# Ascend-Research/HeadPoseEstimation-WHENet

Measured on AMD Instinct MI355X. Metric: head crops/sec (224x224), higher is better.
Workload: dtype f16

## Files before the change

__graft_entry__.py:

```python
from __future__ import annotations

import os
import subprocess
import sys
from concurrent.futures import ThreadPoolExecutor

ROOT = os.path.dirname(os.path.abspath(__file__))
PKG = os.path.join(ROOT, "headposeestimation-whenet_amd")
CSRC = os.path.join(PKG, "csrc")
LIBDIR = os.path.join(PKG, "lib")
OBJDIR = os.path.join(PKG, "build")
LIB = os.path.join(LIBDIR, "libwhenet_hip.so")

SOURCES = ["stem.hip", "stemdw.hip", "dw.hip", "se.hip", "pw.hip", "head.hip", "head7.hip", "front.hip", "front2.hip", "front2s.hip", "front7.hip", "mb7.hip", "frame.hip", "yolo.hip", "convert.hip",
           "snapshot.cpp", "engine.cpp", "engine_post.cpp", "engine_ops.cpp", "capi.cpp"]
HEADERS = ["common.h", "spec.h", "snapshot.h", "kernels.h", "device_math.h", "engine.h", "engine_internal.h", "stamps.h", "se_device.h", "front_tuned_f16.inc", "front_tuned_f32.inc", "front2_tuned.inc", "front2s_tuned.inc",
           os.path.join("..", "..", "include", "whenet_hip.h")]
EXTRA_FLAGS = {"front2.hip": ["-mllvm", "-amdgpu-mfma-vgpr-form"], "front2s.hip": ["-mllvm", "-amdgpu-mfma-vgpr-form"], "front7.hip": ["-mllvm", "-amdgpu-mfma-vgpr-form"],
               "mb7.hip": ["-mllvm", "-amdgpu-mfma-vgpr-form"]}
CXXFLAGS = ["--offload-arch=gfx950", "-mcode-object-version=5", "-O3", "-std=c++17", "-fPIC", "-Wall",
            "-Wno-unused-function", "-fvisibility=hidden"]


def _hipcc() -> str:
    for cand in (os.environ.get("HIPCC"), "/opt/rocm/bin/hipcc", "hipcc"):
        if cand and (os.path.isabs(cand) and os.path.exists(cand) or not os.path.isabs(cand)):
            return cand
    raise RuntimeError("hipcc not found")


def _stale(target: str, deps) -> bool:
    if not os.path.exists(target):
        return True
    t = os.path.getmtime(target)
    return any(os.path.getmtime(d) > t for d in deps if os.path.exists(d))


def build(force: bool = False, verbose: bool = False) -> None:
    os.makedirs(LIBDIR, exist_ok=True)
    os.makedirs(OBJDIR, exist_ok=True)
    hipcc = _hipcc()
    hdrs = [os.path.join(CSRC, h) for h in HEADERS]

    def compile_one(src: str) -> str:
        s = os.path.join(CSRC, src)
        o = os.path.join(OBJDIR, src.replace(".", "_") + ".o")
        if force or _stale(o, [s] + hdrs):
            cmd = [hipcc] + CXXFLAGS + EXTRA_FLAGS.get(src, []) + ["-c", s, "-o", o]
            if verbose:
                print(" ".join(cmd), flush=True)
            r = subprocess.run(cmd, capture_output=True, text=True)
            if r.returncode != 0:
                raise RuntimeError(f"hipcc failed on {src}:\n{r.stdout}\n{r.stderr}")
        return o

    with ThreadPoolExecutor(max_workers=min(8, len(SOURCES))) as ex:
        objs = list(ex.map(compile_one, SOURCES))
    if force or _stale(LIB, objs):
        cmd = [hipcc, "--offload-arch=gfx950", "-shared", "-fPIC", "-o", LIB] + objs + \
              ["-Wl,-rpath,/opt/rocm/lib", "-Wl,--no-undefined"]
        if verbose:
            print(" ".join(cmd), flush=True)
        r = subprocess.run(cmd, capture_output=True, text=True)
        if r.returncode != 0:
            raise RuntimeError(f"link failed:\n{r.stdout}\n{r.stderr}")
    if PKG not in sys.path:
        sys.path.insert(0, PKG)
    import whenet
    from whenet_hip import _lib
    _lib.load()

# ... 55 lines not shown
```

headposeestimation-whenet_amd/csrc/engine.cpp:

```cpp
#include "engine_internal.h"

#include <mutex>

#include <algorithm>
#include <cstdlib>
#include <cmath>
#include <cstring>

namespace whenet {

using namespace detail;

void* Engine::upload_bytes(const void* p, size_t nbytes) {
    void* d = nullptr;
    WHENET_HIP_CHECK(hipMalloc(&d, nbytes ? nbytes : 16));
    weight_allocs_.push_back(d);
    if (nbytes) WHENET_HIP_CHECK(hipMemcpy(d, p, nbytes, hipMemcpyHostToDevice));
    return d;
}

template <typename T> T* Engine::upload(const std::vector<T>& v) {
    return static_cast<T*>(upload_bytes(v.data(), v.size() * sizeof(T)));
}

// ... 36 lines not shown
    for (const HostBlock& hb : m.blocks) {
        DevBlock b;
        b.spec = hb.spec;
        if (hb.spec.has_expand()) b.expand = upload_pw(hb.expand);
        b.dw.k = hb.dw.k;
        b.dw.C = hb.dw.C;
        b.dw.w = upload(hb.dw.w);
        b.dw.bias = upload(hb.dw.bias);
        b.dw.plan = plan_dw(dtype_, hb.spec.k, hb.spec.s, hb.spec.h_in, hb.spec.h_out, hb.dw.C);
        b.se.C = hb.se.C;
        b.se.R = hb.se.R;
        b.se.w1t = upload(hb.se.w1t);
        b.se.b1 = upload(hb.se.b1);
        b.se.w2 = upload(hb.se.w2);
        b.se.w2c = upload(hb.se.w2c);
        b.se.b2 = upload(hb.se.b2);
        if (split_ && !hb.se.excite.packed_split.empty()) {
            b.se.w2p = upload_bytes(hb.se.excite.packed_split.data(), hb.se.excite.packed_split.size());
            b.se.KSr = hb.se.excite.KS_split;
            b.se.w2_wsi = hb.se.excite.wsi;
        } else if (dtype_ == WHENET_F16 && !hb.se.excite.packed.empty()) {
            b.se.w2p = upload_bytes(hb.se.excite.packed.data(), hb.se.excite.packed.size());
            b.se.KSr = hb.se.excite.KS;
        }
        b.project = upload_pw(hb.project);
        partial_per_crop_ = std::max(partial_per_crop_, size_t(b.dw.plan.ntiles()) * b.dw.C);
        if (hb.spec.has_expand()) {
            b.fplan = plan_front(dtype_, hb.spec.k, hb.spec.s, hb.spec.h_in, hb.spec.h_out, hb.dw.C);
            partial_per_crop_ = std::max(partial_per_crop_, size_t(b.fplan.ntiles()) * b.dw.C);
            partial_per_crop_ = std::max(partial_per_crop_, size_t(b.fplan.ntiles()) * size_t(b.fplan.chunks) *
                                                                size_t(se_padded_r(b.se.R)));
            if (dtype_ == WHENET_F16) {
                b.f2plan = plan_front2(hb.spec.k, hb.spec.s, hb.spec.h_in, hb.spec.h_out, hb.dw.C);
                b.f2_preferred = front2_preferred(hb.spec.k, hb.spec.s, hb.spec.h_in, hb.dw.C);
                b.dw.wt = upload(pack_dw_toeplitz(hb.dw.w, hb.spec.k, hb.spec.s, hb.dw.C, b.f2plan.xs));
                partial_per_crop_ = std::max(partial_per_crop_, size_t(b.f2plan.ntiles()) * b.dw.C);
                partial_per_crop_ = std::max(partial_per_crop_, size_t(b.f2plan.ntiles()) * size_t(b.f2plan.chunks) *
                                                                    size_t(se_padded_r(b.se.R)));
            }
            if (split_ && front2s_supported(hb.spec.k, hb.spec.s, hb.spec.h_in, hb.spec.cin)) {
                b.f2s_supported = true;
                b.f2splan = plan_front2s(hb.spec.k, hb.spec.s, hb.spec.h_in, hb.spec.h_out, hb.dw.C, &b.f2s_tm);
                b.f2s_preferred = front2s_preferred(hb.spec.k, hb.spec.s, hb.spec.h_in, hb.dw.C);
                b.dw.wts = upload(pack_dw_toeplitz_s(hb.dw.w, hb.spec.k, hb.spec.s, hb.dw.C, b.f2s_tm, &b.dw.wts_wsi));
                partial_per_crop_ = std::max(partial_per_crop_, size_t(b.f2splan.ntiles()) * size_t(b.f2splan.chunks) *
                                                                    size_t(se_padded_r(b.se.R)));
            }
            b.f7_supported = front7_supported(hb.spec.k, hb.spec.s, hb.spec.h_in, hb.spec.cin);
            if (b.f7_supported) {
                if (dtype_ == WHENET_F16) b.dw.wt7 = upload(pack_dw_toeplitz(hb.dw.w, hb.spec.k, 1, hb.dw.C, 4 - hb.spec.k / 2));
                b.f7_chunks = front7_plan_for(dtype_, hb.spec.cin, hb.dw.C, 64).chunks;
                partial_per_crop_ = std::max(partial_per_crop_, size_t(b.f7_chunks) * size_t(se_padded_r(b.se.R)));
            }
        }
        if (mb7_supported(dtype_, hb.spec.k, hb.spec.s, hb.spec.h_in, hb.spec.cin, hb.dw.C, hb.se.R, hb.spec.cout, hb.spec.has_skip())) {
            std::vector<half_t> w1p, w2p;
            pack_mb7_se(hb.se.w1t, hb.se.w2, hb.se.C, hb.se.R, &w1p, &w2p);
            b.mb7.wds = upload(pack_mb7_taps(hb.dw.w, hb.spec.k, hb.dw.C));
            b.mb7.w1p = upload(w1p);
            b.mb7.w2p = upload(w2p);
            b.mb7.ok = true;
        }
        blocks_.push_back(b);
    }
    head_ = upload_pw(m.head);
    fold12_pw_ = upload_pw(m.fold12);
    d_fold12_w32_ = upload(m.fold12_w32);
    d_dense_w_ = upload(m.dense_w);
    d_dense_b_ = upload(m.dense_b);
    WHENET_HIP_CHECK(hipDeviceSynchronize());
}

void Engine::open_device(int device_id) {
    int count = 0;
    hipError_t e = hipGetDeviceCount(&count);
    if (e != hipSuccess || count <= 0)
        throw Error(WHENET_ENODEV, std::string("no HIP device visible (") + hipGetErrorString(e) +
                                       "); libwhenet_hip has no CPU fallback");
    WHENET_REQUIRE(device_id >= 0 && device_id < count, WHENET_ENODEV,
                   "device_id " + std::to_string(device_id) + " out of range (" + std::to_string(count) + " devices)");
    DeviceGuard guard(device_id);
    WHENET_HIP_CHECK(hipGetDeviceProperties(&prop_, device_id));
    WHENET_REQUIRE(std::strstr(prop_.gcnArchName, "gfx950") != nullptr, WHENET_ENODEV,
                   std::string("device is ") + prop_.gcnArchName + "; this library carries gfx950 code only");
    num_cus_ = prop_.multiProcessorCount;

    WHENET_HIP_CHECK(hipStreamCreateWithFlags(&stream_, hipStreamNonBlocking));
    WHENET_HIP_CHECK(hipEventCreateWithFlags(&fork_ev_, hipEventDisableTiming));
    for (int i = 0; i < MAX_LANES - 1; ++i) {
        hipEvent_t ev = nullptr;
        WHENET_HIP_CHECK(hipEventCreateWithFlags(&ev, hipEventDisableTiming));
        join_ev_.push_back(ev);
    }
}

Engine::Engine(int device_id) : device_(device_id), dtype_(WHENET_F32) { open_device(device_id); }

void Engine::require_model() const {
    WHENET_REQUIRE(has_model_, WHENET_EINVAL, "this handle was created without a network (whenet_create_postproc)");
}

Engine::~Engine() {
    (void)hipSetDevice(device_);
    if (stream_) (void)hipStreamSynchronize(stream_);
    if (copy_stream_) (void)hipStreamSynchronize(copy_stream_);
    for (auto& kv : graphs_) (void)hipGraphExecDestroy(kv.second);
// ... 19 lines not shown
    if (hout_ypr_) (void)hipHostFree(hout_ypr_);
    if (hout_amax_) (void)hipHostFree(hout_amax_);
    if (hout_logits_) (void)hipHostFree(hout_logits_);
    void* arena[] = {x0_, x1_, e_, d_, hc_, partial_, gate_, hcount_, in_u8_, o_ypr_, o_amax_, o_logits_, in_f32_, yolo_scratch_};
    for (void* p : arena)
        if (p) (void)hipFree(p);
    for (void* p : weight_allocs_) (void)hipFree(p);
    for (hipStream_t st : lane_streams_) { (void)hipStreamSynchronize(st); (void)hipStreamDestroy(st); }
    for (hipEvent_t ev : join_ev_) (void)hipEventDestroy(ev);
    if (fork_ev_) (void)hipEventDestroy(fork_ev_);
    if (stream_) (void)hipStreamDestroy(stream_);
    if (copy_stream_) (void)hipStreamDestroy(copy_stream_);
}

void Engine::set_option(const std::string& key, long value) {
    DeviceGuard guard(device_);
    if (key == "graph") {
        use_graph_ = value != 0;
    } else if (key == "pw_impl") {
        WHENET_REQUIRE(value == 0 || value == 1, WHENET_EINVAL, "pw_impl must be 0 (MFMA) or 1 (check kernel)");
        pw_impl_ = int(value);
        sync();
        drop_graphs();
    } else if (key == "fuse_front") {
        fuse_front_ = value != 0;
        sync();
        drop_graphs();
    } else if (key == "se_fuse") {
        WHENET_REQUIRE(value >= 0 && value <= 3, WHENET_EINVAL,
                       "se_fuse must be 0 (never), 1 (where the prologue form pays), 2 (prologue form on every block) or 3 (1 + the matrix-core form on blocks 7-16, default)");
        se_fuse_ = int(value);
        sync();
        drop_graphs();
    } else if (key == "front_impl") {
        WHENET_REQUIRE(value >= 0 && value <= 2, WHENET_EINVAL,
                       "front_impl must be 0 (front.hip everywhere), 1 (per layer, default) or 2 (front2.hip / front2s.hip wherever they exist)");
        front_impl_ = int(value);
        sync();
        drop_graphs();
    } else if (key == "f2s_mask") {
        WHENET_REQUIRE(value >= -1 && value < (1 << 17), WHENET_EINVAL, "f2s_mask must be -1 or a bit mask of blocks 2..12");
        f2s_mask_ = int(value);
        sync();
        drop_graphs();
    } else if (key == "head_fuse") {
        head_fuse_ = value != 0;
        sync();
        drop_graphs();
    } else if (key == "concurrent") {
        xcd_always_ = value != 0;
        sync();
        drop_graphs();
    } else if (key == "xcd_map") {
        WHENET_REQUIRE(value >= 0 && value <= 7, WHENET_EINVAL, "xcd_map must be a bit mask 0..7 (1 = front / front2, 2 = front7, 4 = head7)");
        xcd_map_ = int(value);
        sync();
        drop_graphs();
    } else if (key == "mb7") {
        mb7_ = value != 0;
        sync();
        drop_graphs();
    } else if (key == "front7") {
        front7_ = value != 0;
        sync();
        drop_graphs();
    } else if (key == "fold12") {
        fold12_ = value != 0;
        sync();
        drop_graphs();
    } else if (key == "stem_fuse") {
        stem_fuse_ = value != 0;
        sync();
        drop_graphs();
    } else if (key == "poison") {
        poison_ = value != 0;
    } else if (key == "lanes" || key == "device_lanes") {
        WHENET_REQUIRE(value >= 1 && value <= MAX_LANES, WHENET_EINVAL, "lanes must be 1..8");
        lanes_ = int(value);
        if (key == "lanes") host_lanes_ = int(value);
        sync();
        drop_graphs();
    } else if (key == "split_heads") {
        split_heads_ = value != 0;
        sync();
        drop_graphs();
    } else if (key == "lane_graphs") {
        lane_graphs_ = value != 0;
        sync();
        drop_graphs();
    } else if (key == "pw_staged") {
        pw_staged_ = value != 0;
        sync();
        drop_graphs();
    } else if (key == "split_pw") {
        WHENET_REQUIRE(split_ || value == 0, WHENET_EINVAL, "split_pw: the handle was not created as WHENET_F32S");
        split_pw_ = value != 0;
        sync();
        drop_graphs();
    } else if (key == "host_pinned_max") {
        WHENET_REQUIRE(value >= 0 && value <= 4096, WHENET_EINVAL, "host_pinned_max must be 0..4096");
        sync();
        host_pinned_max_ = int(value);
    } else if (key == "se_fuse_tiny") {
        WHENET_REQUIRE(value >= 0 && value <= 64, WHENET_EINVAL, "se_fuse_tiny must be 0..64");
        se_fuse_tiny_ = int(value);
        sync();
        drop_graphs();
    } else if (key == "host_lanes") {
        WHENET_REQUIRE(value >= 1 && value <= MAX_LANES, WHENET_EINVAL, "host_lanes must be 1..8");
        host_lanes_ = int(value);
    } else if (key == "min_lane_crops") {
        WHENET_REQUIRE(value >= 1, WHENET_EINVAL, "min_lane_crops must be >= 1");
        min_lane_crops_ = int(value);
        sync();
        drop_graphs();
    } else if (key == "repeat") {
// ... 74 lines not shown
    x1_ = alloc(N * X_ELEMS * es);
    e_ = alloc(N * E_ELEMS * es);
    d_ = alloc(N * D_ELEMS * es);
    hc_ = alloc(N * HC_ELEMS * es);
    partial_ = static_cast<float*>(alloc(N * partial_per_crop_ * sizeof(float)));
    gate_ = static_cast<float*>(alloc(N * 1152 * sizeof(float)));
    hcount_ = static_cast<unsigned*>(alloc(N * sizeof(unsigned)));
    WHENET_HIP_CHECK(hipMemsetAsync(hcount_, 0, N * sizeof(unsigned), stream_));
    WHENET_HIP_CHECK(hipStreamSynchronize(stream_));
    in_u8_ = static_cast<uint8_t*>(alloc(N * IN_BYTES));
    o_ypr_ = static_cast<float*>(alloc(N * 3 * sizeof(float)));
    o_amax_ = static_cast<int32_t*>(alloc(N * 3 * sizeof(int32_t)));
    o_logits_ = static_cast<float*>(alloc(N * N_LOGITS * sizeof(float)));
    cap_ = n;
    arena_bytes_ = total;
}

namespace {

struct Rec {
    LaunchRecorder* rec;
    hipStream_t s;
    int repeat = 1;
    template <typename F>
    void operator()(const std::string& layer, const char* kind, const std::string& kernel, double bytes, double flops,
                    F&& fn) {
        if (!rec) {
            for (int i = 0; i < repeat; ++i) fn();
            return;
        }
        if (rec->first_pass) {
            LaunchRecorder::Entry e;
            e.layer = layer;
            e.kind = kind;
            e.kernel = kernel;
            e.bytes = bytes;
            e.flops = flops;
            WHENET_HIP_CHECK(hipEventCreate(&e.stop));
            rec->entries.push_back(e);
        }
        LaunchRecorder::Entry& e = rec->entries.at(rec->cursor++);
        fn();
        WHENET_HIP_CHECK(hipEventRecord(e.stop, s));
    }
};

}

Engine::BlockSchedule Engine::block_schedule(const DevBlock& b, int n) const {
    BlockSchedule r;
    r.fused = fuse_front_ && b.spec.has_expand() && pw_impl_ == 0;
    r.use_f7 = r.fused && front_impl_ == 1 && front7_ && b.f7_supported;
    r.use_mb7 = r.use_f7 && mb7_ && dtype_ == WHENET_F16 && b.mb7.ok;
    r.use_f2 = r.fused && !r.use_f7 && dtype_ == WHENET_F16 && (front_impl_ == 2 || (front_impl_ == 1 && b.f2_preferred));
    const bool f2s_pick = f2s_mask_ >= 0 ? ((f2s_mask_ >> b.spec.index) & 1) != 0 : b.f2s_preferred;
    r.use_f2s = r.fused && !r.use_f7 && split_ && split_pw_ && b.f2s_supported && b.expand.wps != nullptr &&
                (front_impl_ == 2 || (front_impl_ == 1 && f2s_pick));
    r.se_in_front = r.fused;
    r.se_ntiles = r.use_f7 ? 1 : (r.use_f2 ? b.f2plan.ntiles() : (r.use_f2s ? b.f2splan.ntiles() : (r.fused ? b.fplan.ntiles() : b.dw.plan.ntiles())));
    r.se_chunks = r.use_f7 ? b.f7_chunks : (r.use_f2 ? b.f2plan.chunks : (r.use_f2s ? b.f2splan.chunks : b.fplan.chunks));
    const bool se_pays = b.project.K < 320 && r.se_ntiles * r.se_chunks <= 24;
    const bool tiny = !single_stage_call_ && n > 0 && n <= se_fuse_tiny_ && b.project.K < 1152;
    r.se_mfma = r.se_in_front && pw_impl_ == 0 && se_fuse_ == 3 && pw_staged_ && b.project.K >= 320 && b.se.w2p != nullptr &&
                (dtype_ == WHENET_F16 || (split_ && split_pw_));
    r.se_fused = r.se_in_front && pw_impl_ == 0 && (se_fuse_ == 2 || r.se_mfma || ((se_fuse_ == 1 || se_fuse_ == 3) && (se_pays || tiny)));
    return r;
}

bool Engine::fold12_active() const {
    if (!(fold12_ && fuse_front_ && pw_impl_ == 0 && blocks_.size() >= 2)) return false;
    if (dtype_ == WHENET_F16) return front_impl_ == 2 || (front_impl_ == 1 && blocks_[1].f2_preferred);
    const BlockSchedule b2 = block_schedule(blocks_[1]);
    return split_ && split_pw_ && fold12_pw_.wps != nullptr && b2.fused && !b2.use_f2s && !b2.use_f7;
}

bool Engine::stem_fuse_active() const {
    if (!(stem_fuse_ && !blocks_.empty())) return false;
    const DevBlock& b = blocks_[0];
    return !b.spec.has_expand() && !b.spec.has_skip() &&
           stemdw_supported(dtype_, b.dw.plan, b.spec.k, b.spec.s, b.spec.h_in, b.spec.cexp());
}

void* Engine::enqueue_blocks(int first, int last, const View& v, void* cur, int n, hipStream_t s, LaunchRecorder* rec,
                             bool b1_dw_done) {
    const bool fold = fold12_active() && first <= 1 && last >= 2;
    for (int i = first; i <= last; ++i) {
        void* nxt = (cur == v.x0) ? v.x1 : v.x0;
        enqueue_block(blocks_[size_t(i - 1)], v, cur, nxt, n, s, rec, fold && i <= 2 ? i : 0, b1_dw_done && i == 1);
        cur = nxt;
    }
    return cur;
}

void Engine::enqueue_block(const DevBlock& b, const View& v, const void* in, void* out, int n, hipStream_t s,
                           LaunchRecorder* rec, int fold, bool dw_done) {
    Rec R{rec, s, repeat_};
    const BlockSpec& sp = b.spec;
    const std::string p = "b" + std::to_string(sp.index);
    const double es = double(esz());
    const int hw_in = sp.h_in * sp.h_in, hw_out = sp.h_out * sp.h_out;
    const int cexp = sp.cexp();
    const void* dw_in = in;
    const BlockSchedule bs = block_schedule(b, n);
    const bool fused = bs.fused, use_f2 = bs.use_f2, se_in_front = bs.se_in_front, se_fused = bs.se_fused;
    const int se_ntiles = bs.se_ntiles, se_chunks = bs.se_chunks;
    WHENET_REQUIRE(fold == 0 || (fold == 1 && !fused && sp.index == 1) ||
                       (fold == 2 && sp.index == 2 && (use_f2 || (split_ && fused && !bs.use_f2s && !bs.use_f7))), WHENET_EINVAL,
                   "fold12: block outside the folded pair");
    if (bs.use_mb7) {
        WHENET_REQUIRE(fold == 0, WHENET_EINVAL, "mb7: block outside the 7 x 7 stage");
        Mb7Args a{};
        a.x = in;
        a.wep = b.expand.wp;
        a.be = b.expand.bias;
        a.wds = b.mb7.wds;
        a.bd = b.dw.bias;
        a.w1p = b.mb7.w1p;
        a.b1 = b.se.b1;
        a.w2p = b.mb7.w2p;
        a.b2 = b.se.b2;
        a.wpp = b.project.wp;
        a.bp = b.project.bias;
        a.out = out;
        if (single_stage_call_) {
            a.dbg_dw = v.d;
            a.dbg_gate = v.gate;
        }
        a.k = sp.k;
        a.Cout = sp.cout;
        a.skip = sp.has_skip();
        a.n = n;
        R(p + "/mbconv", "mbconv", kernel_name_mb7(sp.k, sp.cout, a.skip).c_str(),
          double(n) * (hw_in * sp.cin * (a.skip ? 2 : 1) + hw_out * sp.cout) * es,
          2.0 * n * (double(hw_in) * sp.cin * cexp + double(hw_out) * sp.k * sp.k * cexp + double(hw_out) * cexp * sp.cout),
          [&] { launch_mb7(a, s); });
        return;
    }
    if (bs.use_f7) {
        Front7Args a{};
        a.dtype = dtype_;
        a.x = in;
        a.wep = b.expand.wp;
        a.be = b.expand.bias;
        a.wdt = dtype_ == WHENET_F16 ? static_cast<const void*>(b.dw.wt7) : static_cast<const void*>(b.dw.w);
        a.bd = b.dw.bias;
        a.out = v.d;
        a.rpart = v.partial;
        a.w1t = b.se.w1t;
        a.R = b.se.R;
        a.k = sp.k;
        a.Cin = sp.cin;
        a.Cexp = cexp;
        a.NTe = b.expand.NTILES;
        a.split = split_ && split_pw_ && b.expand.wps != nullptr;
        a.weps = b.expand.wps;
        a.wsi = b.expand.wsi;
        a.n = n;
        a.xcd_grouped = xcd_grouped(2, n);
        a.plan = front7_plan_for(dtype_, sp.cin, cexp, n);
        R(p + "/front", "front", kernel_name_front7(dtype_, sp.k, a.plan, a.split).c_str(), double(n) * (hw_in * sp.cin + hw_out * cexp) * es,
          2.0 * n * (double(hw_in) * sp.cin * cexp + double(hw_out) * sp.k * sp.k * cexp), [&] { launch_front7(a, s); });
    } else if (use_f2) {
        Front2Args a{};
        a.x = in;
        a.wep = b.expand.wp;
        a.be = b.expand.bias;
        a.wdt = b.dw.wt;
        a.bd = b.dw.bias;
        a.out = v.d;
        a.rpart = v.partial;
        a.w1t = b.se.w1t;
        a.R = b.se.R;
        a.k = sp.k;
        a.s = sp.s;
        a.H = sp.h_in;
        a.Ho = sp.h_out;
        a.Cin = sp.cin;
        a.Cexp = cexp;
        a.pad = sp.pad_before();
        a.KSe = b.expand.KS;
        a.NTe = b.expand.NTILES;
        if (fold == 2) {
            a.wep = d_fold12_w32_;
            a.be = fold12_pw_.bias;
            a.Cin = fold12_pw_.K;
            a.KSe = fold12_pw_.KS;
            a.NTe = fold12_pw_.NTILES;
            a.in_gate = static_cast<const float*>(v.gate);
        }
        a.n = n;
        a.xcd_grouped = xcd_grouped(1, n);
        a.plan = b.f2plan;
        a.plan.threads = front2_threads(b.f2plan, n);
        R(p + "/front", "front", kernel_name_front2(sp.k, sp.s, a.KSe, a.plan.threads, a.plan.xs, a.in_gate != nullptr).c_str(),
          double(n) * (hw_in * a.Cin + hw_out * cexp) * es,
          2.0 * n * (double(hw_in) * a.Cin * cexp + double(hw_out) * sp.k * sp.k * cexp), [&] { launch_front2(a, s); });
    } else if (bs.use_f2s) {
        Front2sArgs a{};
        a.x = in;
        a.weps = b.expand.wps;
        a.be = b.expand.bias;
        a.wdt = b.dw.wts;
        a.bd = b.dw.bias;
        a.out = v.d;
        a.rpart = v.partial;
        a.w1t = b.se.w1t;
        a.R = b.se.R;
        a.k = sp.k;
        a.s = sp.s;
        a.H = sp.h_in;
        a.Ho = sp.h_out;
        a.Cin = sp.cin;
        a.Cexp = cexp;
        a.pad = sp.pad_before();
// ... 668 lines not shown
```

headposeestimation-whenet_amd/csrc/engine.h:

```cpp
#pragma once

#include <map>
#include <memory>
#include <string>
#include <tuple>
#include <vector>

#include "common.h"
#include "kernels.h"
#include "snapshot.h"

namespace whenet {

struct DevPw {
    int K = 0, N = 0, KS = 0, NTILES = 0;
    void* wp = nullptr;
    void* wps = nullptr;
    int KSs = 0;
    float wsi = 1.0f;
    float* wdense = nullptr;
    float* bias = nullptr;
};
struct DevDw {
    int k = 0, C = 0;
    float* w = nullptr;
    float* bias = nullptr;
    half_t* wt = nullptr;
    half_t* wt7 = nullptr;
    float* wts = nullptr;
    float wts_wsi = 1.0f;
    DwPlan plan;
};
struct DevSe {
    int C = 0, R = 0;
    float *w1t = nullptr, *b1 = nullptr, *w2 = nullptr, *b2 = nullptr;
    float* w2c = nullptr;
    void* w2p = nullptr;
    int KSr = 0;
    float w2_wsi = 1.0f;
};
struct DevMb7 {
    bool ok = false;
    half_t *wds = nullptr, *w1p = nullptr, *w2p = nullptr;
};
struct DevBlock {
    BlockSpec spec;
    DevPw expand;
    DevDw dw;
    FrontPlan fplan;
    Front2Plan f2plan;
    bool f2_preferred = false;
    Front2Plan f2splan;
    int f2s_tm = 2;
    bool f2s_supported = false, f2s_preferred = false;
    bool f7_supported = false;
    int f7_chunks = 1;
    DevSe se;
    DevPw project;
    DevMb7 mb7;
};

struct LaunchRecorder {
    struct Entry {
        std::string layer, kind, kernel;
        double bytes = 0, flops = 0;
        hipEvent_t stop = nullptr;
        double total_ms = 0;
    };
    std::vector<Entry> entries;
    hipEvent_t start = nullptr;
    size_t cursor = 0;
    bool first_pass = true;
};

constexpr int MAX_LANES = 8;

class Engine {
  public:
    Engine(const void* snapshot, size_t nbytes, int device_id, int dtype);
    explicit Engine(int device_id);
    ~Engine();
    Engine(const Engine&) = delete;
    Engine& operator=(const Engine&) = delete;

    void set_option(const std::string& key, long value);
    void get_info(whenet_info_t* out) const;

    void forward_host(const uint8_t* crops, int n, float* ypr, int32_t* argmax, float* logits);
    void forward_host_f32(const float* x, int n, float* ypr, int32_t* argmax, float* logits);
    void forward_device(const uint8_t* d_crops, int n, float* d_ypr, int32_t* d_argmax, float* d_logits,
                        hipStream_t stream);
    void sync();
    void release_aux_streams();
    int submit(const uint8_t* crops, int n, int stage = 0, int want_lanes = 0, hipStream_t copy_on = nullptr, hipEvent_t copy_after = nullptr);
    hipStream_t copy_stream_handle();
    hipEvent_t copied_event(int ticket) const;
    void abandon_submissions();
    bool has_pending() const {
        for (const Slot& s : slots_)
            if (s.busy) return true;
        return false;
    }
    int submit_frame(const uint8_t* frame, int fh, int fw, int swap_rb, const int32_t* rects, int k);
    void op_crop_resize(const uint8_t* frame, int fh, int fw, int swap_rb, const int32_t* rects, int k,
                        uint8_t* crops_out);
    void collect(int ticket, float* ypr, int32_t* argmax, float* logits);
    int profile(const uint8_t* d_crops, int n, int iters, whenet_launch_stat_t* stats, int cap);

    void op_stem(const uint8_t* crops, int n, float* out);
// ... 12 lines not shown
    void d2h(void* d, const void* s, size_t nbytes);

    std::string last_error;

  private:
    struct Slot {
        int capacity = 0, n = 0, ticket = -1;
        bool busy = false;
        uint8_t* h_in = nullptr;
        uint8_t* d_in = nullptr;
        float *h_ypr = nullptr, *d_ypr = nullptr;
        int32_t *h_amax = nullptr, *d_amax = nullptr;
        float *h_logits = nullptr, *d_logits = nullptr;
        hipEvent_t copied = nullptr, done = nullptr;
        size_t frame_cap = 0;
        uint8_t *h_frame = nullptr, *d_frame = nullptr;
        int plan_cap = 0;
        int32_t *h_plan = nullptr, *d_plan = nullptr;
    };

    template <typename T> T* upload(const std::vector<T>& v);
    void* upload_bytes(const void* p, size_t nbytes);
    DevPw upload_pw(const HostPw& h);
    void set_split(PwArgs& a, const DevPw& w) const {
        a.staged = pw_staged_;
        a.split = split_ && split_pw_ && w.wps != nullptr;
        a.wps = w.wps;
        a.KSs = w.KSs;
        a.wsi = w.wsi;
    }
    bool split_ = false;
    bool split_pw_ = true;
    bool pw_staged_ = true;
    void ensure_capacity(int n);
    void release_arena();
    void drop_graphs();
    size_t esz() const { return dtype_ == WHENET_F16 ? 2 : 4; }

    struct View {
        void *x0, *x1, *e, *d, *hc;
        float *partial, *gate;
        unsigned* hcount;
    };
    View view(int crop_off) const;
    void enqueue_forward(const View& v, const uint8_t* d_in, int n, float* d_ypr, int32_t* d_amax, float* d_logits,
                         hipStream_t s, LaunchRecorder* rec, const float* d_in_f32 = nullptr);
    void enqueue_block(const DevBlock& b, const View& v, const void* in, void* out, int n, hipStream_t s,
                       LaunchRecorder* rec, int fold = 0, bool dw_done = false);
    void* enqueue_blocks(int first, int last, const View& v, void* cur, int n, hipStream_t s, LaunchRecorder* rec,
                         bool b1_dw_done = false);
    bool stem_fuse_active() const;
    bool fold12_active() const;
    struct BlockSchedule {
        bool fused = false, use_f2 = false, use_f2s = false, use_f7 = false, se_in_front = false, se_fused = false, se_mfma = false;
        bool use_mb7 = false;
        int se_ntiles = 1, se_chunks = 1;
    };
    BlockSchedule block_schedule(const DevBlock& b, int n = 0) const;
    int se_fuse_tiny_ = 0;
    int f2s_mask_ = -1;
    bool single_stage_call_ = false;
    int lanes_for(int n, int want) const;
    void enqueue_lanes(const uint8_t* d_in, int n, float* d_ypr, int32_t* d_amax, float* d_logits, hipStream_t s, int want = 0);
    void run_forward(const uint8_t* d_in, int n, float* d_ypr, int32_t* d_amax, float* d_logits, hipStream_t s, int want = 0);
    void ensure_slot(Slot& s, int n);
    hipStream_t lane_stream(int i);
    using GraphKey = std::tuple<int, int, const void*, void*, void*, void*>;
    template <typename F>
    hipGraphExec_t cached_graph(const GraphKey& key, hipStream_t s, F&& fn);
    void sync_streams(hipStream_t s);
    hipStream_t copy_stream();
    void ensure_slot_frame(Slot& s, size_t frame_bytes, int k);
    Slot* free_slot();

    void open_device(int device_id);
    void require_model() const;
    bool has_model_ = false;
    int device_ = 0, dtype_ = WHENET_F32, num_cus_ = 256;
    bool use_graph_ = true;
    int pw_impl_ = 0;
    int repeat_ = 1;
    bool split_heads_ = true;
    bool fuse_front_ = true;
    int se_fuse_ = 1;
    int front_impl_ = 1;
    bool poison_ = false;
    bool head_fuse_ = true;
    bool front7_ = true;
    bool mb7_ = false;
    int xcd_map_ = 7;
    bool xcd_always_ = false;
    bool xcd_grouped(int bit, int n) const {
        return (xcd_map_ & bit) != 0 && (xcd_always_ || n >= 128);
    }
    bool stem_fuse_ = true;
    bool fold12_ = true;
    int lanes_ = 2;
    bool lane_graphs_ = false;
    int min_lane_crops_ = 16;
    int host_lanes_ = 2;
    std::vector<hipStream_t> lane_streams_;
    std::vector<hipEvent_t> join_ev_;
    hipEvent_t fork_ev_ = nullptr;
    hipStream_t stream_ = nullptr, copy_stream_ = nullptr;
    hipDeviceProp_t prop_{};
    int64_t params_backbone_ = 0, params_heads_ = 0;
    int n_tensors_ = 0;

    std::vector<void*> weight_allocs_;
    float *d_lut_ = nullptr, *d_stem_w_ = nullptr, *d_stem_b_ = nullptr;
    StemDwTable* d_stemdw_tab_ = nullptr;
    std::vector<DevBlock> blocks_;
    DevPw head_;
    DevPw fold12_pw_;
    float* d_fold12_w32_ = nullptr;
    float *d_dense_w_ = nullptr, *d_dense_b_ = nullptr;

    int cap_ = 0;
    size_t arena_bytes_ = 0;
    void *x0_ = nullptr, *x1_ = nullptr, *e_ = nullptr, *d_ = nullptr, *hc_ = nullptr;
    float *partial_ = nullptr, *gate_ = nullptr;
    unsigned* hcount_ = nullptr;
    uint8_t* in_u8_ = nullptr;
    float* in_f32_ = nullptr;
    int in_f32_cap_ = 0;
    float* o_ypr_ = nullptr;
    int32_t* o_amax_ = nullptr;
    float* o_logits_ = nullptr;
    size_t partial_per_crop_ = 0;
    unsigned char* yolo_scratch_ = nullptr;
    size_t yolo_scratch_bytes_ = 0;
    std::vector<int> yolo_counts_;

    std::map<GraphKey, hipGraphExec_t> graphs_;

    Slot slots_[WHENET_MAX_INFLIGHT];
    Slot host_slot_;
    float* hout_ypr_ = nullptr;
    int32_t* hout_amax_ = nullptr;
    float* hout_logits_ = nullptr;
    int hout_cap_ = 0;
// ... 7 lines not shown
```

headposeestimation-whenet_amd/csrc/kernels.h:

```cpp
#pragma once

#include <string>
#include <vector>

#include "common.h"

namespace whenet {

struct StemArgs {
    const uint8_t* in;
    void* out;
    const float* w;
    const float* bias;
    const float* lut;
    int n;
    const float* in_f32 = nullptr;
};
void launch_stem(const StemArgs& a, int dtype, hipStream_t stream);

struct DwPlan {
    int threads = 256;
    int CV = 1;
    int TH = 1;
    int NSX = 1;
// ... 209 lines not shown
    const void* wdt;
    const float* bd;
    void* out;
    float* rpart;
    const float* w1t;
    int R;
    int k, s, H, Ho, Cin, Cexp, pad, KSe, NTe, n;
    float wsi = 1.0f;
    float wsi_d = 1.0f;
    int tm = 2;
    bool pre = false;
    Front2Plan plan;
};
bool front2s_supported(int k, int s, int H, int Cin);
bool front2s_preferred(int k, int s, int H, int Cexp);
Front2Plan make_front2s_plan(int k, int s, int Ho, int Cexp, int CC, int TH, int TXG, int threads);
Front2Plan plan_front2s(int k, int s, int H, int Ho, int Cexp, int* tm);
std::vector<Front2Plan> plan_front2s_candidates(int k, int s, int Ho, int Cexp);
std::vector<float> pack_dw_toeplitz_s(const std::vector<float>& w, int k, int s, int C, int tm, float* wsi);
void launch_front2s(const Front2sArgs& a, hipStream_t stream);
std::string kernel_name_front2s(int k, int s, int kse, int threads, int tm, bool pre);

struct Front7Plan {
    int threads = 512;
    int G = 4;
    int CC = 64;
    int chunks = 1;
    int off_w = 0, off_stage = 0, off_red = 0, off_sum = 0;
    size_t lds_bytes = 0;
};
Front7Plan make_front7_plan(int dtype, int Cin, int Cexp, int G, int CC, int threads);
Front7Plan front7_plan_for(int dtype, int Cin, int Cexp, int n);
bool front7_supported(int k, int s, int H, int Cin);
struct Front7Args {
    int dtype = WHENET_F16;
    const void* x;
    const void* wep;
    const float* be;
    const void* wdt;
    const float* bd;
    void* out;
    float* rpart;
    const float* w1t;
    int R;
    int k, Cin, Cexp, NTe, n;
    Front7Plan plan;
    bool split = false;
    const void* weps = nullptr;
    float wsi = 1.0f;
    bool xcd_grouped = false;
};
void launch_front7(const Front7Args& a, hipStream_t stream);
std::string kernel_name_front7(int dtype, int k, const Front7Plan& p, bool split = false);

struct Mb7Args {
    const void* x;
    const void* wep;
    const float* be;
    const void* wds;
    const float* bd;
    const void* w1p;
    const float* b1;
    const void* w2p;
    const float* b2;
    const void* wpp;
    const float* bp;
    void* out;
    void* dbg_dw = nullptr;
    void* dbg_gate = nullptr;
    int k, Cout, n;
    bool skip;
};
bool mb7_supported(int dtype, int k, int s, int H, int Cin, int Cexp, int R, int Cout, bool skip);
std::vector<half_t> pack_mb7_taps(const std::vector<float>& w , int k, int C);
void pack_mb7_se(const std::vector<float>& w1t , const std::vector<float>& w2 , int C, int R,
                 std::vector<half_t>* w1p, std::vector<half_t>* w2p);
void launch_mb7(const Mb7Args& a, hipStream_t stream);
std::string kernel_name_mb7(int k, int Cout, bool skip);

struct YoloLayer {
    const float* feats;
    int gh, gw;
    int first;
    float anchor[3][2];
};
struct YoloArgs {
    YoloLayer layer[3];
    int num_layers, num_classes, na;
    int N, NP;
    float input_h, input_w, image_h, image_w;
    float off_y, off_x, scale_y, scale_x;
    float score_thr, iou_thr;
    int max_boxes;
    float* boxes;
    float* all_scores;
    int* counts;
    unsigned long long* keys;
    float* out_boxes;
    float* out_scores;
    int* out_index;
    int* out_count;
};
void launch_yolo_eval(const YoloArgs& a, hipStream_t stream);
int yolo_max_select();

constexpr int CROP_PLAN_INTS = 8 + 6 * IMG;
// ... 15 lines not shown
```

Before: 161,000.

## Add fused expand+depthwise+SE-reduce kernel for 14x14 stride-1 blocks in f16

Adds a new front14 HIP kernel for f16 blocks on 14x14 maps with 3x3/5x5 stride-1 depthwise convs and Cin 80 or 112. In one launch it runs the 1x1 expand conv with 32x32 MFMA into LDS, the depthwise conv with 4x4x4 MFMA, swish, and the squeeze-excite reduce partials. The scheduler prefers it over front2 and front2s for eligible blocks, with the aim of removing intermediate global traffic and kernel launches. The cost is high LDS use of up to 160 KB per block, which can limit occupancy, and it adds more template instantiations.

```diff
diff --git a/__graft_entry__.py b/__graft_entry__.py
--- a/__graft_entry__.py
+++ b/__graft_entry__.py
@@ -12,11 +12,12 @@
 OBJDIR = os.path.join(PKG, "build")
 LIB = os.path.join(LIBDIR, "libwhenet_hip.so")
 
-SOURCES = ["stem.hip", "stemdw.hip", "dw.hip", "se.hip", "pw.hip", "head.hip", "head7.hip", "front.hip", "front2.hip", "front2s.hip", "front7.hip", "mb7.hip", "frame.hip", "yolo.hip", "convert.hip",
+SOURCES = ["stem.hip", "stemdw.hip", "dw.hip", "se.hip", "pw.hip", "head.hip", "head7.hip", "front.hip", "front2.hip", "front2s.hip", "front7.hip", "front14.hip", "mb7.hip", "frame.hip", "yolo.hip", "convert.hip",
            "snapshot.cpp", "engine.cpp", "engine_post.cpp", "engine_ops.cpp", "capi.cpp"]
 HEADERS = ["common.h", "spec.h", "snapshot.h", "kernels.h", "device_math.h", "engine.h", "engine_internal.h", "stamps.h", "se_device.h", "front_tuned_f16.inc", "front_tuned_f32.inc", "front2_tuned.inc", "front2s_tuned.inc",
            os.path.join("..", "..", "include", "whenet_hip.h")]
 EXTRA_FLAGS = {"front2.hip": ["-mllvm", "-amdgpu-mfma-vgpr-form"], "front2s.hip": ["-mllvm", "-amdgpu-mfma-vgpr-form"], "front7.hip": ["-mllvm", "-amdgpu-mfma-vgpr-form"],
+               "front14.hip": ["-mllvm", "-amdgpu-mfma-vgpr-form"],
                "mb7.hip": ["-mllvm", "-amdgpu-mfma-vgpr-form"]}
 CXXFLAGS = ["--offload-arch=gfx950", "-mcode-object-version=5", "-O3", "-std=c++17", "-fPIC", "-Wall",
             "-Wno-unused-function", "-fvisibility=hidden"]
diff --git a/headposeestimation-whenet_amd/csrc/engine.cpp b/headposeestimation-whenet_amd/csrc/engine.cpp
--- a/headposeestimation-whenet_amd/csrc/engine.cpp
+++ b/headposeestimation-whenet_amd/csrc/engine.cpp
@@ -112,6 +112,11 @@
                 b.f7_chunks = front7_plan_for(dtype_, hb.spec.cin, hb.dw.C, 64).chunks;
                 partial_per_crop_ = std::max(partial_per_crop_, size_t(b.f7_chunks) * size_t(se_padded_r(b.se.R)));
             }
+        }
+        if (dtype_ == WHENET_F16 && hb.spec.has_expand() && front14_supported(hb.spec.k, hb.spec.s, hb.spec.h_in, hb.spec.cin, hb.dw.C)) {
+            b.f14_supported = true;
+            b.f14_chunks = front14_plan_for(hb.spec.cin, hb.dw.C, 64).chunks;
+            partial_per_crop_ = std::max(partial_per_crop_, size_t(b.f14_chunks) * size_t(se_padded_r(b.se.R)));
         }
         if (mb7_supported(dtype_, hb.spec.k, hb.spec.s, hb.spec.h_in, hb.spec.cin, hb.dw.C, hb.se.R, hb.spec.cout, hb.spec.has_skip())) {
             std::vector<half_t> w1p, w2p;
@@ -237,7 +242,7 @@
         sync();
         drop_graphs();
     } else if (key == "xcd_map") {
-        WHENET_REQUIRE(value >= 0 && value <= 7, WHENET_EINVAL, "xcd_map must be a bit mask 0..7 (1 = front / front2, 2 = front7, 4 = head7)");
+        WHENET_REQUIRE(value >= 0 && value <= 7, WHENET_EINVAL, "xcd_map must be a bit mask 0..7 (1 = front / front2, 2 = front7 / front14, 4 = head7)");
         xcd_map_ = int(value);
         sync();
         drop_graphs();
@@ -247,6 +252,10 @@
         drop_graphs();
     } else if (key == "front7") {
         front7_ = value != 0;
+        sync();
+        drop_graphs();
+    } else if (key == "front14") {
+        front14_ = value != 0;
         sync();
         drop_graphs();
     } else if (key == "fold12") {
@@ -427,13 +436,14 @@
     r.fused = fuse_front_ && b.spec.has_expand() && pw_impl_ == 0;
     r.use_f7 = r.fused && front_impl_ == 1 && front7_ && b.f7_supported;
     r.use_mb7 = r.use_f7 && mb7_ && dtype_ == WHENET_F16 && b.mb7.ok;
-    r.use_f2 = r.fused && !r.use_f7 && dtype_ == WHENET_F16 && (front_impl_ == 2 || (front_impl_ == 1 && b.f2_preferred));
+    r.use_f14 = r.fused && dtype_ == WHENET_F16 && front_impl_ == 1 && front14_ && b.f14_supported;
+    r.use_f2 = r.fused && !r.use_f7 && !r.use_f14 && dtype_ == WHENET_F16 && (front_impl_ == 2 || (front_impl_ == 1 && b.f2_preferred));
     const bool f2s_pick = f2s_mask_ >= 0 ? ((f2s_mask_ >> b.spec.index) & 1) != 0 : b.f2s_preferred;
     r.use_f2s = r.fused && !r.use_f7 && split_ && split_pw_ && b.f2s_supported && b.expand.wps != nullptr &&
                 (front_impl_ == 2 || (front_impl_ == 1 && f2s_pick));
     r.se_in_front = r.fused;
-    r.se_ntiles = r.use_f7 ? 1 : (r.use_f2 ? b.f2plan.ntiles() : (r.use_f2s ? b.f2splan.ntiles() : (r.fused ? b.fplan.ntiles() : b.dw.plan.ntiles())));
-    r.se_chunks = r.use_f7 ? b.f7_chunks : (r.use_f2 ? b.f2plan.chunks : (r.use_f2s ? b.f2splan.chunks : b.fplan.chunks));
+    r.se_ntiles = (r.use_f7 || r.use_f14) ? 1 : (r.use_f2 ? b.f2plan.ntiles() : (r.use_f2s ? b.f2splan.ntiles() : (r.fused ? b.fplan.ntiles() : b.dw.plan.ntiles())));
+    r.se_chunks = r.use_f7 ? b.f7_chunks : r.use_f14 ? b.f14_chunks : (r.use_f2 ? b.f2plan.chunks : (r.use_f2s ? b.f2splan.chunks : b.fplan.chunks));
     const bool se_pays = b.project.K < 320 && r.se_ntiles * r.se_chunks <= 24;
     const bool tiny = !single_stage_call_ && n > 0 && n <= se_fuse_tiny_ && b.project.K < 1152;
     r.se_mfma = r.se_in_front && pw_impl_ == 0 && se_fuse_ == 3 && pw_staged_ && b.project.K >= 320 && b.se.w2p != nullptr &&
@@ -535,6 +545,26 @@
         a.plan = front7_plan_for(dtype_, sp.cin, cexp, n);
         R(p + "/front", "front", kernel_name_front7(dtype_, sp.k, a.plan, a.split).c_str(), double(n) * (hw_in * sp.cin + hw_out * cexp) * es,
           2.0 * n * (double(hw_in) * sp.cin * cexp + double(hw_out) * sp.k * sp.k * cexp), [&] { launch_front7(a, s); });
+    } else if (bs.use_f14) {
+        Front14Args a{};
+        a.x = in;
+        a.wep = b.expand.wp;
+        a.be = b.expand.bias;
+        a.wdt = b.dw.wt;
+        a.bd = b.dw.bias;
+        a.out = v.d;
+        a.rpart = v.partial;
+        a.w1t = b.se.w1t;
+        a.R = b.se.R;
+        a.k = sp.k;
+        a.Cin = sp.cin;
+        a.Cexp = cexp;
+        a.NTe = b.expand.NTILES;
+        a.n = n;
+        a.xcd_grouped = xcd_grouped(2, n);
+        a.plan = front14_plan_for(sp.cin, cexp, n);
+        R(p + "/front", "front", kernel_name_front14(sp.k, sp.cin, a.plan).c_str(), double(n) * (hw_in * sp.cin + hw_out * cexp) * es,
+          2.0 * n * (double(hw_in) * sp.cin * cexp + double(hw_out) * sp.k * sp.k * cexp), [&] { launch_front14(a, s); });
     } else if (use_f2) {
         Front2Args a{};
         a.x = in;
diff --git a/headposeestimation-whenet_amd/csrc/engine.h b/headposeestimation-whenet_amd/csrc/engine.h
--- a/headposeestimation-whenet_amd/csrc/engine.h
+++ b/headposeestimation-whenet_amd/csrc/engine.h
@@ -55,6 +55,8 @@
     bool f2s_supported = false, f2s_preferred = false;
     bool f7_supported = false;
     int f7_chunks = 1;
+    bool f14_supported = false;
+    int f14_chunks = 1;
     DevSe se;
     DevPw project;
     DevMb7 mb7;
@@ -173,7 +175,8 @@
     bool stem_fuse_active() const;
     bool fold12_active() const;
     struct BlockSchedule {
-        bool fused = false, use_f2 = false, use_f2s = false, use_f7 = false, se_in_front = false, se_fused = false, se_mfma = false;
+        bool fused = false, use_f2 = false, use_f2s = false, use_f7 = false, use_f14 = false, se_in_front = false, se_fused = false,
+             se_mfma = false;
         bool use_mb7 = false;
         int se_ntiles = 1, se_chunks = 1;
     };
@@ -208,6 +211,7 @@
     bool poison_ = false;
     bool head_fuse_ = true;
     bool front7_ = true;
+    bool front14_ = true;
     bool mb7_ = false;
     int xcd_map_ = 7;
     bool xcd_always_ = false;
diff --git a/headposeestimation-whenet_amd/csrc/front14.hip b/headposeestimation-whenet_amd/csrc/front14.hip
--- /dev/null
+++ b/headposeestimation-whenet_amd/csrc/front14.hip
@@ -0,0 +1,384 @@
+#include "device_math.h"
+#include "kernels.h"
+#include "stamps.h"
+
+#include <atomic>
+#include <cstdlib>
+#include <string>
+#include <type_traits>
+
+namespace whenet {
+
+namespace {
+
+constexpr int HW14 = 14;
+constexpr int RW14 = 20;
+constexpr int RPB14 = RW14 * 2;
+constexpr int CPB14 = 608;
+constexpr int PX14 = 28;
+
+struct F14Params {
+    const half_t* x;
+    const half8* wep;
+    const float* be;
+    const half4* wdt;
+    const float* bd;
+    half_t* out;
+    float* rpart;
+    const float* w1t;
+    int n, Cexp, NTe, R, RPse;
+    int off_w, off_stage, off_red, off_sum;
+    int chunks, ngroups, xcd;
+};
+
+template <int K, int KS, int G, int CC, int NTHR>
+__global__ __launch_bounds__(NTHR) void whenet_front14_kernel(const F14Params p) {
+    constexpr int NWAVE = NTHR / 64;
+    constexpr int PAD = K / 2;
+    constexpr int NT = CC / 32, NCB = CC / 16;
+    constexpr int SPC = 7;
+    constexpr int nstrip = G * SPC;
+    constexpr int SPW = (nstrip + NWAVE - 1) / NWAVE;
+    constexpr int ROWB = KS * 32;
+    constexpr int SPB = ROWB + 16;
+    constexpr int NV = PX14 * ROWB / 16;
+    constexpr int NVL = (NV + 63) / 64;
+
+    extern __shared__ __attribute__((aligned(16))) unsigned char smem[];
+    unsigned char* E = smem;
+    const half8* Wl = reinterpret_cast<const half8*>(smem + p.off_w);
+
+    const int tid = threadIdx.x;
+    const int lane = tid & 63;
+    const int wave = __builtin_amdgcn_readfirstlane(tid >> 6);
+    const int g = lane >> 5, lm = lane & 31;
+    int grp, chunk;
+    xcd_unit(int(blockIdx.x), p.ngroups, p.chunks, grp, chunk, p.xcd != 0);
+    const int c0 = chunk * CC;
+    const int crop0 = grp * G;
+    const int nlast = p.n - 1;
+
+    STAMP(0);
+    constexpr int nwv = KS * NT * 64;
+    constexpr int WV = (nwv + NTHR - 1) / NTHR;
+    half8 wstage[WV];
+#pragma unroll
+    for (int i = 0; i < WV; ++i) {
+        const int v = tid + i * NTHR;
+        if (v < nwv) {
+            const int ks = v / (NT * 64), r = v - ks * (NT * 64);
+            wstage[i] = p.wep[(size_t(ks) * p.NTe + (c0 >> 5)) * 64 + r];
+        }
+    }
+    const unsigned char* xb = reinterpret_cast<const unsigned char*>(p.x);
+    half8 raw[SPW][NVL];
+#pragma unroll
+    for (int r = 0; r < SPW; ++r) {
+        const int s = wave + r * NWAVE;
+        if (s < nstrip) {
+            const int cr = s / SPC, sr = s - cr * SPC;
+            const int gc = crop0 + cr < nlast ? crop0 + cr : nlast;
+            const unsigned char* src = xb + (size_t(gc) * (HW14 * HW14) + size_t(sr) * PX14) * ROWB;
+#pragma unroll
+            for (int i = 0; i < NVL; ++i) {
+                const int v = i * 64 + lane < NV ? i * 64 + lane : NV - 1;
+                raw[r][i] = *reinterpret_cast<const half8*>(src + v * 16);
+            }
+        }
+    }
+    float bias_t[NT];
+#pragma unroll
+    for (int t = 0; t < NT; ++t) bias_t[t] = p.be[c0 + t * 32 + lm];
+    constexpr int nitem = G * NCB * 2;
+    const int cl = lane >> 2, j = lane & 3;
+    half4 A[K][2];
+    float bdv = 0.f;
+    auto load_taps = [&](int it) {
+        const int cb = (it >> 1) % NCB;
+        const half4* src = p.wdt + size_t((c0 >> 4) + cb) * K * 2 * 64 + lane;
+#pragma unroll
+        for (int ky = 0; ky < K; ++ky) {
+            A[ky][0] = src[(ky * 2) * 64];
+            A[ky][1] = src[(ky * 2 + 1) * 64];
+        }
+        bdv = p.bd[c0 + cb * 16 + cl];
+    };
+    int it = wave;
+    if (it < nitem) load_taps(it);
+
+    half8 a[SPW][KS];
+    {
+        unsigned char* sa = E + wave * (PX14 * SPB);
+        const int slot = lm & 15;
+        int px = slot - PAD;
+        px = px < 0 ? 0 : (px > HW14 - 1 ? HW14 - 1 : px);
+        const int pf = (lm >> 4) * HW14 + px;
+#pragma unroll
+        for (int r = 0; r < SPW; ++r) {
+            if (wave + r * NWAVE < nstrip) {
+#pragma unroll
+                for (int i = 0; i < NVL; ++i) {
+                    const int v = i * 64 + lane;
+                    if (v < NV) {
+                        const int q = v / (ROWB / 16);
+                        *reinterpret_cast<half8*>(sa + q * SPB + (v - q * (ROWB / 16)) * 16) = raw[r][i];
+                    }
+                }
+#pragma unroll
+                for (int ks = 0; ks < KS; ++ks) a[r][ks] = *reinterpret_cast<const half8*>(sa + pf * SPB + ks * 32 + g * 16);
+            }
+        }
+    }
+    {
+        half8* dst = reinterpret_cast<half8*>(smem + p.off_w);
+#pragma unroll
+        for (int i = 0; i < WV; ++i) {
+            const int v = tid + i * NTHR;
+            if (v < nwv) dst[v] = wstage[i];
+        }
+    }
+    lds_barrier();
+    STAMP(1);
+
+#pragma unroll
+    for (int r = 0; r < SPW; ++r) {
+        const int s = wave + r * NWAVE;
+        if (s >= nstrip) break;
+        const int cr = s / SPC, sr = s - cr * SPC;
+#pragma unroll
+        for (int t = 0; t < NT; ++t) {
+            float16v acc;
+#pragma unroll
+            for (int q = 0; q < 16; ++q) acc[q] = bias_t[t];
+#pragma unroll
+            for (int ks = 0; ks < KS; ++ks)
+                acc = __builtin_amdgcn_mfma_f32_32x32x16_f16(a[r][ks], Wl[(ks * NT + t) * 64 + lane], acc, 0, 0, 0);
+            unsigned char* ep = E + (cr * CC + t * 32 + lm) * CPB14 + (2 * sr) * RPB14;
+#pragma unroll
+            for (int qq = 0; qq < 4; ++qq) {
+                const float2v y0 = swish2(float2v{acc[4 * qq], acc[4 * qq + 1]});
+                const float2v y1 = swish2(float2v{acc[4 * qq + 2], acc[4 * qq + 3]});
+                const float y[4] = {y0[0], y0[1], y1[0], y1[1]};
+                half4 o;
+#pragma unroll
+                for (int i = 0; i < 4; ++i) {
+                    const bool lo = (qq & 1) == 0 && i < PAD;
+                    const bool hi = (qq & 1) == 1 && 4 + i >= 6 + PAD;
+                    o[i] = ((lo && g == 0) || (hi && g == 1)) ? half_t(0) : half_t(y[i]);
+                }
+                unsigned char* rp = ep + (qq >> 1) * RPB14;
+                *reinterpret_cast<half4*>(rp + (2 * (qq & 1) + g) * 8) = o;
+                if ((qq & 1) && g) *reinterpret_cast<half4*>(rp + 32) = half4{0, 0, 0, 0};
+            }
+        }
+    }
+    STAMP(2);
+
+    constexpr int W1Q = CC / 16;
+    float4v w1v[W1Q];
+    {
+        const int jo = (tid >> 2) & 63, q = tid & 3;
+        const float* wrow = p.w1t + size_t(jo < p.R ? jo : p.R - 1) * p.Cexp + c0 + q * (CC / 4);
+#pragma unroll
+        for (int i = 0; i < W1Q; ++i) w1v[i] = *reinterpret_cast<const float4v*>(wrow + 4 * i);
+    }
+    lds_barrier();
+    STAMP(3);
+
+    unsigned char* stg = smem + p.off_stage + wave * 2048;
+    float* s_red = reinterpret_cast<float*>(smem + p.off_red);
+    float* s_sum = reinterpret_cast<float*>(smem + p.off_sum);
+    const int jP = (lane >> 1) & 3, iP = (lane >> 3) & 3, hP = lane & 1, rP = lane >> 5;
+    const unsigned row_bytes = unsigned(HW14) * unsigned(p.Cexp) * 2u;
+
+    for (; it < nitem; it += NWAVE) {
+        const int seg = it & 1, cbq = it >> 1, cb = cbq % NCB, cr = cbq / NCB;
+        const int c = cb * 16 + cl;
+        const unsigned char* bp = E + (cr * CC + c) * CPB14 + j * 8;
+        float4v acc[7];
+#pragma unroll
+        for (int q = 0; q < 7; ++q) acc[q] = float4v{bdv, bdv, bdv, bdv};
+        auto sweep = [&](auto segc) {
+            constexpr int SEG = decltype(segc)::value;
+            constexpr int r0 = SEG * 7 - PAD;
+#pragma unroll
+            for (int ir = (r0 < 0 ? 0 : r0); ir <= (r0 + 6 + K - 1 > HW14 - 1 ? HW14 - 1 : r0 + 6 + K - 1); ++ir) {
+                const half4 b0 = *reinterpret_cast<const half4*>(bp + ir * RPB14);
+                const half4 b1 = *reinterpret_cast<const half4*>(bp + ir * RPB14 + 8);
+#pragma unroll
+                for (int ky = 0; ky < K; ++ky) {
+                    const int d = ir - r0 - ky;
+                    if (d >= 0 && d < 7) {
+                        acc[d] = __builtin_amdgcn_mfma_f32_4x4x4f16(A[ky][0], b0, acc[d], 0, 0, 0);
+                        acc[d] = __builtin_amdgcn_mfma_f32_4x4x4f16(A[ky][1], b1, acc[d], 0, 0, 0);
+                    }
+                }
+            }
+        };
+        if (seg == 0) sweep(std::integral_constant<int, 0>{});
+        else sweep(std::integral_constant<int, 1>{});
+        if (it + NWAVE < nitem) load_taps(it + NWAVE);
+        const bool okc = crop0 + cr < p.n;
+        float m[4];
+#pragma unroll
+        for (int i = 0; i < 4; ++i) m[i] = (okc && 4 * j + i < HW14) ? 1.f : 0.f;
+        const int oxP = 4 * jP + iP;
+        const bool okP = okc && oxP < HW14;
+        unsigned char* outb = reinterpret_cast<unsigned char*>(p.out + size_t(okc ? crop0 + cr : 0) * (HW14 * HW14) * p.Cexp);
+        const unsigned obase = (unsigned(seg * 7 + rP) * unsigned(HW14) + unsigned(oxP)) * unsigned(p.Cexp) * 2u +
+                               unsigned(c0 + cb * 16 + hP * 8) * 2u;
+        float2v sum2 = {0.f, 0.f};
+        const float2v m01 = {m[0], m[1]}, m23 = {m[2], m[3]};
+        unsigned char* sw = stg + j * 32 + cl * 2;
+#pragma unroll
+        for (int half = 0; half < 2; ++half) {
+            const int q0 = half * 4, nr = half ? 3 : 4;
+#pragma unroll
+            for (int q = 0; q < nr; ++q) {
+                const float2v y01 = swish2(float2v{acc[q0 + q][0], acc[q0 + q][1]});
+                const float2v y23 = swish2(float2v{acc[q0 + q][2], acc[q0 + q][3]});
+                sum2 = y01 * m01 + sum2;
+                sum2 = y23 * m23 + sum2;
+                *reinterpret_cast<half_t*>(sw + (q * 4 + 0) * 128) = half_t(y01[0]);
+                *reinterpret_cast<half_t*>(sw + (q * 4 + 1) * 128) = half_t(y01[1]);
+                *reinterpret_cast<half_t*>(sw + (q * 4 + 2) * 128) = half_t(y23[0]);
+                *reinterpret_cast<half_t*>(sw + (q * 4 + 3) * 128) = half_t(y23[1]);
+            }
+            wave_lds_sync();
+#pragma unroll
+            for (int pp = 0; pp < 2; ++pp) {
+                const int rl = 2 * pp + rP;
+                const half8 v = *reinterpret_cast<const half8*>(stg + (pp * 64 + lane) * 16);
+                if (okP && rl < nr) *reinterpret_cast<half8*>(outb + obase + unsigned(q0 + 2 * pp) * row_bytes) = v;
+            }
+            wave_lds_sync();
+        }
+        float sum = sum2[0] + sum2[1];
+        sum += quad_xor1(sum);
+        sum += quad_xor2(sum);
+        if (j == 0) s_red[(cr * 2 + seg) * CC + c] = sum;
+    }
+    STAMP(4);
+    lds_barrier();
+    STAMP(5);
+
+#pragma unroll
+    for (int i0 = 0; i0 < G * CC; i0 += NTHR) {
+        const int i = i0 + tid;
+        if (i < G * CC) {
+            const int cr = i / CC, cc = i % CC;
+            float t = 0.0f;
+            t += s_red[(cr * 2) * CC + cc];
+            t += s_red[(cr * 2 + 1) * CC + cc];
+            s_sum[i] = t;
+        }
+    }
+    lds_barrier();
+    {
+        const int jo = (tid >> 2) & 63, q = tid & 3;
+        for (int cr = tid >> 8; cr < G; cr += NTHR / 256) {
+            float accr = 0.0f;
+            if (jo < p.R) {
+                const float* sp = s_sum + cr * CC + q * (CC / 4);
+#pragma unroll
+                for (int i = 0; i < W1Q; ++i) {
+                    const float4v sv = *reinterpret_cast<const float4v*>(sp + 4 * i);
+#pragma unroll
+                    for (int e = 0; e < 4; ++e) accr = fmaf(sv[e], w1v[i][e], accr);
+                }
+            }
+            const float pair = accr + quad_xor1(accr);
+            const float tot = pair + quad_xor2(pair);
+            if (q == 0 && jo < p.RPse && crop0 + cr < p.n)
+                p.rpart[(size_t(crop0 + cr) * p.chunks + chunk) * p.RPse + jo] = (jo < p.R) ? tot : 0.0f;
+        }
+    }
+    STAMP(6);
+}
+
+struct OncePerDevice14 {
+    std::atomic<bool> done[64];
+    OncePerDevice14() { for (auto& d : done) d.store(false, std::memory_order_relaxed); }
+};
+
+template <int K, int KS, int G, int CC, int NTHR>
+void launch_f14(const Front14Args& a, hipStream_t stream) {
+    const Front14Plan& pl = a.plan;
+    F14Params p{};
+    p.x = static_cast<const half_t*>(a.x);
+    p.wep = static_cast<const half8*>(a.wep);
+    p.be = a.be;
+    p.wdt = static_cast<const half4*>(a.wdt);
+    p.bd = a.bd;
+    p.out = static_cast<half_t*>(a.out);
+    p.rpart = a.rpart;
+    p.w1t = a.w1t;
+    p.n = a.n;  p.Cexp = a.Cexp;  p.NTe = a.NTe;
+    p.R = a.R;  p.RPse = (a.R + 3) & ~3;
+    p.off_w = pl.off_w;  p.off_stage = pl.off_stage;  p.off_red = pl.off_red;  p.off_sum = pl.off_sum;
+    WHENET_REQUIRE(pl.lds_bytes <= 160 * 1024, WHENET_EINVAL, "front14: the tile plan needs more than 160 KB of LDS");
+    static OncePerDevice14 attr;
+    int dev = 0;
+    WHENET_HIP_CHECK(hipGetDevice(&dev));
+    auto kern = &whenet_front14_kernel<K, KS, G, CC, NTHR>;
+    if (dev >= 0 && dev < 64 && !attr.done[dev].load(std::memory_order_acquire)) {
+        WHENET_HIP_CHECK(hipFuncSetAttribute(reinterpret_cast<const void*>(kern), hipFuncAttributeMaxDynamicSharedMemorySize, 160 * 1024));
+        attr.done[dev].store(true, std::memory_order_release);
+    }
+    p.chunks = pl.chunks;  p.ngroups = ceil_div(a.n, pl.G);  p.xcd = a.xcd_grouped ? 1 : 0;
+    hipLaunchKernelGGL(kern, dim3(unsigned(p.chunks) * unsigned(p.ngroups)), dim3(NTHR), pl.lds_bytes, stream, p);
+    WHENET_HIP_CHECK(hipGetLastError());
+}
+
+}
+
+Front14Plan make_front14_plan(int Cin, int Cexp, int G, int CC, int threads) {
+    WHENET_REQUIRE(threads == 512 && (G == 1 || G == 2) && CC == 96 && Cexp % CC == 0 && (Cin == 80 || Cin == 112), WHENET_EINVAL,
+                   "front14: bad tile plan");
+    Front14Plan p;
+    p.threads = threads;
+    p.G = G;
+    p.CC = CC;
+    p.chunks = Cexp / CC;
+    const int nwave = threads / 64, ks = Cin / 16, nt = CC / 32;
+    const int e_bytes = G * CC * CPB14;
+    const int strip_waves = G * 7 < nwave ? G * 7 : nwave;
+    WHENET_REQUIRE(strip_waves * PX14 * (Cin * 2 + 16) <= e_bytes, WHENET_EINVAL, "front14: the input stage does not fit the tile");
+    p.off_w = e_bytes;
+    const int w_bytes = ks * nt * 1024, stage_bytes = nwave * 2048;
+    p.off_stage = p.off_w;
+    p.off_red = p.off_w + (w_bytes > stage_bytes ? w_bytes : stage_bytes);
+    p.off_sum = p.off_red + G * 2 * CC * 4;
+    p.lds_bytes = size_t(p.off_sum) + size_t(G) * CC * 4;
+    return p;
+}
+
+Front14Plan front14_plan_for(int Cin, int Cexp, int n) {
+    (void)n;
+    static const int G = [] { const char* e = getenv("WHENET_FRONT14_G"); return e && atoi(e) == 2 ? 2 : 1; }();
+    return make_front14_plan(Cin, Cexp, G, 96, 512);
+}
+
+bool front14_supported(int k, int s, int H, int Cin, int Cexp) {
+    return (k == 3 || k == 5) && s == 1 && H == HW14 && (Cin == 80 || Cin == 112) && Cexp % 96 == 0;
+}
+
+void launch_front14(const Front14Args& a, hipStream_t stream) {
+    WHENET_REQUIRE(front14_supported(a.k, 1, HW14, a.Cin, a.Cexp) && a.w1t != nullptr && a.R >= 1 && a.R <= 64 && a.n >= 1,
+                   WHENET_EINVAL, "front14: 14 x 14 maps, 3x3 / 5x5 stride-1 kernels, Cin = 80 | 112, squeeze-excite reduce conv in the kernel");
+    const int key = (a.k * 100 + a.Cin / 16) * 10 + a.plan.G;
+    switch (key) {
+#define F14_CASE(K, KS, G) case (K * 100 + KS) * 10 + G: launch_f14<K, KS, G, 96, 512>(a, stream); break;
+        F14_CASE(3, 5, 1) F14_CASE(5, 5, 1) F14_CASE(5, 7, 1)
+        F14_CASE(3, 5, 2) F14_CASE(5, 5, 2) F14_CASE(5, 7, 2)
+#undef F14_CASE
+        default: throw Error(WHENET_EINVAL, "front14: no instantiation for this (kernel, Cin, G) plan");
+    }
+}
+
+std::string kernel_name_front14(int k, int cin, const Front14Plan& p) {
+    return "whenet_front14_kernel<" + std::to_string(k) + ", " + std::to_string(cin / 16) + ", " + std::to_string(p.G) + ", " +
+           std::to_string(p.CC) + ", " + std::to_string(p.threads) + ">";
+}
+
+}
diff --git a/headposeestimation-whenet_amd/csrc/kernels.h b/headposeestimation-whenet_amd/csrc/kernels.h
--- a/headposeestimation-whenet_amd/csrc/kernels.h
+++ b/headposeestimation-whenet_amd/csrc/kernels.h
@@ -285,6 +285,34 @@
 };
 void launch_front7(const Front7Args& a, hipStream_t stream);
 std::string kernel_name_front7(int dtype, int k, const Front7Plan& p, bool split = false);
+
+struct Front14Plan {
+    int threads = 512;
+    int G = 1;
+    int CC = 96;
+    int chunks = 1;
+    int off_w = 0, off_stage = 0, off_red = 0, off_sum = 0;
+    size_t lds_bytes = 0;
+};
+Front14Plan make_front14_plan(int Cin, int Cexp, int G, int CC, int threads);
+Front14Plan front14_plan_for(int Cin, int Cexp, int n);
+bool front14_supported(int k, int s, int H, int Cin, int Cexp);
+struct Front14Args {
+    const void* x;
+    const void* wep;
+    const float* be;
+    const void* wdt;
+    const float* bd;
+    void* out;
+    float* rpart;
+    const float* w1t;
+    int R;
+    int k, Cin, Cexp, NTe, n;
+    Front14Plan plan;
+    bool xcd_grouped = false;
+};
+void launch_front14(const Front14Args& a, hipStream_t stream);
+std::string kernel_name_front14(int k, int cin, const Front14Plan& p);
 
 struct Mb7Args {
     const void* x;
```

Measured after the change: 163,100 (median of 6 runs). 1.3% higher.
